# SebastianHafner/greedy_multimodal_learning

Measured on AMD Instinct MI355X. Metric: multi-view images/sec + step ms, ModelNet40 2-view MVCNN+MMTM @1/2/4/8 GPU, higher is better.
Workload: dtype bf16; 1 GPU; C2: 2-view MVCNN(ResNet-18 x2)+MMTM x3, guided gating (training_guided.gin eps 0.01, window 5, unlocked; decided on bf16-trunk gradients: d_BDR within ~6.5e-3 of eps may decide unlike fp32, INTEGRATION.md section 3); params=23773008, global_batch=64, per_gpu_batch=64, image=224, parallelism=dp1, hipgraph=True, device_gate=True

## Files before the change

greedy_multimodal_learning_amd/csrc/maxpool.hip:

```cpp
#include <type_traits>

#include "gm_common.h"

namespace gm {
namespace {

template <typename E>
__device__ __forceinline__ float round_to(float v) {
    if constexpr (std::is_same<E, uint16_t>::value) return __uint_as_float((uint32_t)Elem<uint16_t>::f2bf(v) << 16);
    else return v;
}

struct PoolArgs {
    int N, H, W, C8;
    int P, Q, k, s, pad;
    FastDiv fd_c8, fd_q, fd_p, fd_w, fd_h, fd_s;
    FastDiv fd_ng;
};

template <typename E, bool BNRELU = false>
__global__ __launch_bounds__(256) void k_maxpool_fwd(PoolArgs a, const void* __restrict__ x, void* __restrict__ y,
                                                     uint2* __restrict__ idx, const float* __restrict__ coef = nullptr,
                                                     void* __restrict__ xsel = nullptr) {
    const unsigned total = (unsigned)a.N * a.P * a.Q * a.C8;
    for (unsigned i = blockIdx.x * 256 + threadIdx.x; i < total; i += gridDim.x * 256) {
        unsigned t = a.fd_c8.div(i);
        const int cg = (int)(i - t * a.C8);
        unsigned t2 = a.fd_q.div(t);
        const int q = (int)(t - t2 * a.Q);
        const unsigned n_ = a.fd_p.div(t2);
        const int p = (int)(t2 - n_ * a.P);
        const int n = (int)n_;
        const int h0 = p * a.s - a.pad, w0 = q * a.s - a.pad;
        float m[8], xs[8];
        uint32_t ix[8];
        float sc[8], sh[8];
        if (BNRELU) {
            const float* cf = coef + (size_t)a.fd_ng.div((unsigned)n) * (a.C8 * 16);
            const float4* c4 = reinterpret_cast<const float4*>(cf + cg * 8);
            const float4* s4 = reinterpret_cast<const float4*>(cf + a.C8 * 8 + cg * 8);
            const float4 c0 = c4[0], c1 = c4[1], s0 = s4[0], s1 = s4[1];
            sc[0] = c0.x; sc[1] = c0.y; sc[2] = c0.z; sc[3] = c0.w; sc[4] = c1.x; sc[5] = c1.y; sc[6] = c1.z; sc[7] = c1.w;
            sh[0] = s0.x; sh[1] = s0.y; sh[2] = s0.z; sh[3] = s0.w; sh[4] = s1.x; sh[5] = s1.y; sh[6] = s1.z; sh[7] = s1.w;
        }
        const int hs = h0 < 0 ? 0 : h0, ws = w0 < 0 ? 0 : w0;
        const uint32_t first = (uint32_t)((hs - h0) * a.k + (ws - w0));
#pragma unroll
        for (int j = 0; j < 8; ++j) {
            m[j] = -__builtin_huge_valf();
            xs[j] = 0.f;
            ix[j] = first;
        }
        if (a.k == 3) {
            float v[9][8];
            const int xc = ((n * a.H + hs) * a.W + ws) * a.C8 + cg;
            const int x00 = xc + ((h0 - hs) * a.W + (w0 - ws)) * a.C8;
            const int WC8 = a.W * a.C8;
#pragma unroll
            for (int u = 0; u < 9; ++u) {
                const int h = h0 + u / 3, w = w0 + u % 3;
                const bool in = h >= 0 && h < a.H && w >= 0 && w < a.W;
                V8<E>::ld(x, in ? x00 + (u / 3) * WC8 + (u % 3) * a.C8 : xc, v[u]);
            }
#pragma unroll
            for (int u = 0; u < 9; ++u) {
                const int h = h0 + u / 3, w = w0 + u % 3;
                if (h < 0 || h >= a.H || w < 0 || w >= a.W) continue;
#pragma unroll
                for (int j = 0; j < 8; ++j) {
                    const float z = BNRELU ? round_to<E>(relu_nan(fmaf(v[u][j], sc[j], sh[j]))) : v[u][j];
                    if (z > m[j] || __builtin_isnan(z)) {
                        m[j] = z;
                        xs[j] = v[u][j];
                        ix[j] = (uint32_t)u;
                    }
                }
            }
        } else
        for (int r = 0; r < a.k; ++r) {
            const int h = h0 + r;
            if (h < 0 || h >= a.H) continue;
            for (int c = 0; c < a.k; ++c) {
                const int w = w0 + c;
                if (w < 0 || w >= a.W) continue;
                float v[8], raw[8];
                V8<E>::ld(x, (((long long)n * a.H + h) * a.W + w) * a.C8 + cg, v);
#pragma unroll
                for (int j = 0; j < 8; ++j) raw[j] = v[j];
                if (BNRELU) {
#pragma unroll
                    for (int j = 0; j < 8; ++j) v[j] = round_to<E>(relu_nan(fmaf(v[j], sc[j], sh[j])));
                }
                const uint32_t pos = (uint32_t)(r * a.k + c);
#pragma unroll
                for (int j = 0; j < 8; ++j) {
                    if (v[j] > m[j] || __builtin_isnan(v[j])) {
                        m[j] = v[j];
                        xs[j] = raw[j];
                        ix[j] = pos;
                    }
                }
            }
        }
        V8<E>::st(y, i, m);
        if (xsel) V8<E>::st(xsel, i, xs);
        idx[i] = make_uint2(ix[0] | ix[1] << 8 | ix[2] << 16 | ix[3] << 24, ix[4] | ix[5] << 8 | ix[6] << 16 | ix[7] << 24);
    }
}

template <typename E>
__global__ __launch_bounds__(256) void k_maxpool_bwd(PoolArgs a, const void* __restrict__ dy,
                                                     const uint2* __restrict__ idx, void* __restrict__ dx) {
    const unsigned total = (unsigned)a.N * a.H * a.W * a.C8;
    for (unsigned i = blockIdx.x * 256 + threadIdx.x; i < total; i += gridDim.x * 256) {
        unsigned t = a.fd_c8.div(i);
        const int cg = (int)(i - t * a.C8);
        unsigned t2 = a.fd_w.div(t);
        const int w = (int)(t - t2 * a.W);
        const unsigned n_ = a.fd_h.div(t2);
        const int h = (int)(t2 - n_ * a.H);
        const int n = (int)n_;
        int plo = h + a.pad - a.k + 1;
        plo = plo <= 0 ? 0 : (int)a.fd_s.div((unsigned)(plo + a.s - 1));
        int phi = (int)a.fd_s.div((unsigned)(h + a.pad));
        if (phi > a.P - 1) phi = a.P - 1;
        int qlo = w + a.pad - a.k + 1;
        qlo = qlo <= 0 ? 0 : (int)a.fd_s.div((unsigned)(qlo + a.s - 1));
        int qhi = (int)a.fd_s.div((unsigned)(w + a.pad));
        if (qhi > a.Q - 1) qhi = a.Q - 1;
        float g[8];
#pragma unroll
        for (int j = 0; j < 8; ++j) g[j] = 0.f;
        if (a.k == 3 && a.s == 2) {
            uint2 iv[4];
            float dv[4][8];
            bool ok[4];
            uint32_t pos[4];
#pragma unroll
            for (int u = 0; u < 4; ++u) {
                const int p = phi - 1 + (u >> 1), q = qhi - 1 + (u & 1);
                ok[u] = p >= plo && q >= qlo;
                const int pc = ok[u] ? p : phi, qc = ok[u] ? q : qhi;
                const long long o = (((long long)n * a.P + pc) * a.Q + qc) * a.C8 + cg;
                iv[u] = idx[o];
                V8<E>::ld(dy, o, dv[u]);
                pos[u] = (uint32_t)((h - (p * a.s - a.pad)) * a.k + (w - (q * a.s - a.pad)));
            }
#pragma unroll
            for (int u = 0; u < 4; ++u)
#pragma unroll
                for (int j = 0; j < 8; ++j) {
                    const uint32_t b = ((j < 4 ? iv[u].x : iv[u].y) >> (8 * (j & 3))) & 0xffu;
                    if (ok[u] && b == pos[u]) g[j] += dv[u][j];
                }
            V8<E>::st(dx, i, g);
            continue;
        }
        for (int p = plo; p <= phi; ++p) {
            for (int q = qlo; q <= qhi; ++q) {
                const long long o = (((long long)n * a.P + p) * a.Q + q) * a.C8 + cg;
                const uint2 iv = idx[o];
                const uint32_t pos = (uint32_t)((h - (p * a.s - a.pad)) * a.k + (w - (q * a.s - a.pad)));
                float d[8];
                V8<E>::ld(dy, o, d);
#pragma unroll
                for (int j = 0; j < 8; ++j) {
                    const uint32_t b = ((j < 4 ? iv.x : iv.y) >> (8 * (j & 3))) & 0xffu;
                    if (b == pos) g[j] += d[j];
                }
            }
        }
        V8<E>::st(dx, i, g);
    }
}

int prep(const gm_pool_desc* d, PoolArgs& a, const char* fn) {
    if (!d) {
        set_error("%s: null descriptor", fn);
        return GM_E_ARG;
    }
    if (d->N <= 0 || d->H <= 0 || d->W <= 0 || d->C <= 0 || d->C % 8 || d->k < 1 || d->k > 15 || d->stride < 1 ||
        d->pad < 0 || 2 * d->pad > d->k) {
        set_error("%s: unsupported N=%d H=%d W=%d C=%d k=%d s=%d pad=%d (C%%8==0, k<=15, pad<=k/2)", fn, d->N, d->H,
                  d->W, d->C, d->k, d->stride, d->pad);
        return GM_E_ARG;
    }
    a.N = d->N; a.H = d->H; a.W = d->W; a.C8 = d->C / 8;
    a.k = d->k; a.s = d->stride; a.pad = d->pad;
    a.P = (d->H + 2 * d->pad - d->k) / d->stride + 1;
    a.Q = (d->W + 2 * d->pad - d->k) / d->stride + 1;
    if (a.P <= 0 || a.Q <= 0) {
        set_error("%s: empty output", fn);
        return GM_E_ARG;
    }
    if ((long long)a.N * a.H * a.W * a.C8 >= (1ll << 31)) {
        set_error("%s: tensor too large (N*H*W*C/8 >= 2^31)", fn);
        return GM_E_ARG;
    }
    a.fd_c8 = FastDiv((uint32_t)a.C8);
    a.fd_q = FastDiv((uint32_t)a.Q);
    a.fd_p = FastDiv((uint32_t)a.P);
    a.fd_w = FastDiv((uint32_t)a.W);
    a.fd_h = FastDiv((uint32_t)a.H);
    a.fd_s = FastDiv((uint32_t)a.s);
    a.fd_ng = FastDiv((uint32_t)a.N);
    return GM_OK;
}

inline int grid_for(long long n) {
    long long g = (n + 255) / 256;
    if (g > 16384) g = 16384;
    return (int)(g < 1 ? 1 : g);
}

}
}

using namespace gm;

template <typename E>
int pool_fwd(const gm_pool_desc* d, const void* x, void* y, void* idx, void* stream, const char* fn) {
    PoolArgs a;
    int rc = prep(d, a, fn);
    if (rc) return rc;
    GM_REQUIRE(x && y && idx, "%s: null pointer", fn);
    const long long n = (long long)a.N * a.P * a.Q * a.C8;
    hipLaunchKernelGGL(k_maxpool_fwd<E>, dim3(grid_for(n)), dim3(256), 0, as_stream(stream), a, x, y,
                       static_cast<uint2*>(idx));
    return check_launch("k_maxpool_fwd");
}

template <typename E>
int pool_bwd(const gm_pool_desc* d, const void* dy, const void* idx, void* dx, void* stream, const char* fn) {
    PoolArgs a;
    int rc = prep(d, a, fn);
    if (rc) return rc;
    GM_REQUIRE(dy && idx && dx, "%s: null pointer", fn);
    const long long n = (long long)a.N * a.H * a.W * a.C8;
    hipLaunchKernelGGL(k_maxpool_bwd<E>, dim3(grid_for(n)), dim3(256), 0, as_stream(stream), a, dy,
                       static_cast<const uint2*>(idx), dx);
    return check_launch("k_maxpool_bwd");
}

extern "C" int gm_maxpool2d_fwd_bf16(const gm_pool_desc* d, const void* x, void* y, void* idx, void* stream) {
    return pool_fwd<uint16_t>(d, x, y, idx, stream, "gm_maxpool2d_fwd_bf16");
}

extern "C" int gm_bn_relu_maxpool2d_fwd_grouped_bf16(const gm_pool_desc* d, int G, const void* x, const float* coef,
                                                     void* y, void* idx, void* xsel, void* stream) {
    const char* fn = "gm_bn_relu_maxpool2d_fwd_grouped_bf16";
    GM_REQUIRE(d && G >= 1 && G <= 64, "%s: 1..64 groups", fn);
    gm_pool_desc dg = *d;
    dg.N = d->N * G;
    PoolArgs a;
    int rc = prep(&dg, a, fn);
    if (rc) return rc;
    a.fd_ng = FastDiv((uint32_t)d->N);
    GM_REQUIRE(x && coef && y && idx, "%s: null pointer", fn);
    const long long n = (long long)a.N * a.P * a.Q * a.C8;
    hipLaunchKernelGGL((k_maxpool_fwd<uint16_t, true>), dim3(grid_for(n)), dim3(256), 0, as_stream(stream), a, x, y,
                       static_cast<uint2*>(idx), coef, xsel);
    return check_launch("k_maxpool_fwd<bnrelu>");
}

extern "C" int gm_bn_relu_maxpool2d_fwd_bf16(const gm_pool_desc* d, const void* x, const float* coef, void* y,
                                             void* idx, void* stream) {
    return gm_bn_relu_maxpool2d_fwd_grouped_bf16(d, 1, x, coef, y, idx, nullptr, stream);
}

extern "C" int gm_maxpool2d_bwd_bf16(const gm_pool_desc* d, const void* dy, const void* idx, void* dx, void* stream) {
    return pool_bwd<uint16_t>(d, dy, idx, dx, stream, "gm_maxpool2d_bwd_bf16");
}

extern "C" int gm_maxpool2d_fwd_f32(const gm_pool_desc* d, const void* x, void* y, void* idx, void* stream) {
    return pool_fwd<float>(d, x, y, idx, stream, "gm_maxpool2d_fwd_f32");
}

extern "C" int gm_maxpool2d_bwd_f32(const gm_pool_desc* d, const void* dy, const void* idx, void* dx, void* stream) {
    return pool_bwd<float>(d, dy, idx, dx, stream, "gm_maxpool2d_bwd_f32");
}
```

Before: 36860 view-images/s.

## Add banded row-reuse kernel for fused BN-ReLU 3x3/s2 stem maxpool

Adds a specialized kernel for the fused BN+ReLU+maxpool forward (k=3, s=2, pad=1). Each thread handles a band of four output rows and carries the bottom input row of one output over as the top row of the next, which cuts redundant loads and normalization work. Comparisons are done on packed bf16 values with integer max and bit-select instructions, and a scalar exact path handles NaN and inf. The cost is fewer threads, since parallelism drops by the band factor, plus reliance on the bit patterns of non-negative bf16 values after ReLU for the ordering and tie-break to match the generic kernel.

```diff
diff --git a/greedy_multimodal_learning_amd/csrc/maxpool.hip b/greedy_multimodal_learning_amd/csrc/maxpool.hip
--- a/greedy_multimodal_learning_amd/csrc/maxpool.hip
+++ b/greedy_multimodal_learning_amd/csrc/maxpool.hip
@@ -108,6 +108,183 @@
     }
 }
 
+constexpr int kPoolBand = 4;
+
+struct RowArgs {
+    PoolArgs p;
+    int nb;
+    unsigned total;
+    FastDiv fd_nb;
+};
+
+typedef unsigned short us2 __attribute__((ext_vector_type(2)));
+typedef float f2 __attribute__((ext_vector_type(2)));
+typedef __bf16 bf2 __attribute__((ext_vector_type(2)));
+constexpr uint32_t kOne2 = 0x00010001u;
+
+__device__ __forceinline__ uint32_t pk_max(uint32_t a, uint32_t b) {
+    return __builtin_bit_cast(uint32_t,
+                              __builtin_elementwise_max(__builtin_bit_cast(us2, a), __builtin_bit_cast(us2, b)));
+}
+__device__ __forceinline__ uint32_t pk_sub(uint32_t a, uint32_t b) {
+    const us2 d = __builtin_bit_cast(us2, a) - __builtin_bit_cast(us2, b);
+    return __builtin_bit_cast(uint32_t, d);
+}
+__device__ __forceinline__ uint32_t pk_eq(uint32_t m1, uint32_t z) {
+    uint32_t r;
+    asm("v_pk_ashrrev_i16 %0, %1, %2" : "=v"(r) : "s"(15u * kOne2), "v"(pk_sub(m1, z)));
+    return r;
+}
+__device__ __forceinline__ uint32_t pk_sel(uint32_t mask, uint32_t a, uint32_t b) {
+    uint32_t r;
+    asm("v_bfi_b32 %0, %1, %2, %3" : "=v"(r) : "v"(mask), "v"(a), "v"(b));
+    return r;
+}
+
+struct RowRes {
+    uint32_t m[4], x[4], c[4];
+};
+
+__device__ __forceinline__ void rows_norm(const uint4 u, const f2* sc, const f2* sh, uint32_t* z) {
+    const uint32_t w[4] = {u.x, u.y, u.z, u.w};
+#pragma unroll
+    for (int k = 0; k < 4; ++k) {
+        f2 v = {bf_lo(w[k]), bf_hi(w[k])};
+        v = __builtin_elementwise_fma(v, sc[k], sh[k]);
+        v.x = relu_nan(v.x);
+        v.y = relu_nan(v.y);
+        z[k] = __builtin_bit_cast(uint32_t, __builtin_convertvector(v, bf2));
+    }
+}
+
+__device__ __forceinline__ void rows_scan(const uint4* v, uint32_t cl2, uint32_t cr2, const f2* sc, const f2* sh,
+                                          RowRes& r) {
+    uint32_t z0[4], z1[4], z2[4];
+    rows_norm(v[0], sc, sh, z0);
+    rows_norm(v[1], sc, sh, z1);
+    rows_norm(v[2], sc, sh, z2);
+    const uint32_t x0[4] = {v[0].x, v[0].y, v[0].z, v[0].w};
+    const uint32_t x1[4] = {v[1].x, v[1].y, v[1].z, v[1].w};
+    const uint32_t x2[4] = {v[2].x, v[2].y, v[2].z, v[2].w};
+#pragma unroll
+    for (int k = 0; k < 4; ++k) {
+        const uint32_t m = pk_max(pk_max(z0[k], z1[k]), z2[k]);
+        const uint32_t m1 = pk_sub(m, kOne2);
+        const uint32_t e0 = pk_eq(m1, z0[k]), e1 = pk_eq(m1, z1[k]);
+        r.m[k] = m;
+        r.x[k] = pk_sel(e0, x0[k], pk_sel(e1, x1[k], x2[k]));
+        r.c[k] = pk_sel(e0, cl2, pk_sel(e1, kOne2, cr2));
+    }
+}
+
+__device__ __forceinline__ void rows_window_exact(const PoolArgs& a, const uint4* __restrict__ x, int n, int p, int q,
+                                               int cg, const f2* sc, const f2* sh, uint32_t* mz, uint32_t* mx,
+                                               uint32_t* mpos) {
+    const int h0 = 2 * p - 1, w0 = 2 * q - 1;
+    const uint32_t first = (h0 < 0 ? 3u : 0u) + (w0 < 0 ? 1u : 0u);
+    float m[8], xr[8];
+    uint32_t ix[8];
+#pragma unroll
+    for (int j = 0; j < 8; ++j) {
+        m[j] = -__builtin_huge_valf();
+        xr[j] = 0.f;
+        ix[j] = first;
+    }
+#pragma unroll 1
+    for (int u = 0; u < 9; ++u) {
+        const int r = u / 3, c = u - 3 * r;
+        const int h = h0 + r, w = w0 + c;
+        if (h < 0 || h >= a.H || w < 0 || w >= a.W) continue;
+        float v[8];
+        V8<uint16_t>::ld(x, ((n * a.H + h) * a.W + w) * a.C8 + cg, v);
+#pragma unroll
+        for (int j = 0; j < 8; ++j) {
+            const float z = round_to<uint16_t>(relu_nan(fmaf(v[j], sc[j >> 1][j & 1], sh[j >> 1][j & 1])));
+            if (z > m[j] || __builtin_isnan(z)) {
+                m[j] = z;
+                xr[j] = v[j];
+                ix[j] = (uint32_t)u;
+            }
+        }
+    }
+#pragma unroll
+    for (int k = 0; k < 4; ++k) {
+        mz[k] = pack_bf2(m[2 * k], m[2 * k + 1]);
+        mx[k] = pack_bf2(xr[2 * k], xr[2 * k + 1]);
+        mpos[k] = ix[2 * k] | ix[2 * k + 1] << 16;
+    }
+}
+
+__global__ __launch_bounds__(256) void k_stem_pool_rows(RowArgs ra, const uint4* __restrict__ x,
+                                                        uint4* __restrict__ y, uint2* __restrict__ idx,
+                                                        const float* __restrict__ coef, uint4* __restrict__ xsel) {
+    const PoolArgs& a = ra.p;
+    const unsigned i = blockIdx.x * 256 + threadIdx.x;
+    if (i >= ra.total) return;
+    unsigned t = a.fd_c8.div(i);
+    const int cg = (int)(i - t * a.C8);
+    unsigned t2 = a.fd_q.div(t);
+    const int q = (int)(t - t2 * a.Q);
+    const unsigned n_ = ra.fd_nb.div(t2);
+    const int p0 = (int)(t2 - n_ * ra.nb) * kPoolBand;
+    const int p1 = p0 + kPoolBand < a.P ? p0 + kPoolBand : a.P;
+    const int n = (int)n_;
+    f2 sc[4], sh[4];
+    {
+        const float* cf = coef + (size_t)a.fd_ng.div((unsigned)n) * (a.C8 * 16);
+        const float4* c4 = reinterpret_cast<const float4*>(cf + cg * 8);
+        const float4* s4 = reinterpret_cast<const float4*>(cf + a.C8 * 8 + cg * 8);
+        const float4 c0 = c4[0], c1 = c4[1], s0 = s4[0], s1 = s4[1];
+        sc[0] = f2{c0.x, c0.y}; sc[1] = f2{c0.z, c0.w}; sc[2] = f2{c1.x, c1.y}; sc[3] = f2{c1.z, c1.w};
+        sh[0] = f2{s0.x, s0.y}; sh[1] = f2{s0.z, s0.w}; sh[2] = f2{s1.x, s1.y}; sh[3] = f2{s1.z, s1.w};
+    }
+    const bool vl = q > 0, vr = 2 * q + 1 < a.W;
+    const uint32_t cl2 = vl ? 0u : kOne2, cr2 = vr ? 2u * kOne2 : kOne2;
+    const int WC8 = a.W * a.C8;
+    const int oc = n * a.H * WC8 + 2 * q * a.C8 + cg;
+    const int ol = vl ? oc - a.C8 : oc, orr = vr ? oc + a.C8 : oc;
+
+    RowRes top;
+    bool tv = p0 > 0;
+    {
+        const int rb = (tv ? 2 * p0 - 1 : 0) * WC8;
+        const uint4 v[3] = {x[ol + rb], x[oc + rb], x[orr + rb]};
+        rows_scan(v, cl2, cr2, sc, sh, top);
+    }
+    int o = ((n * a.P + p0) * a.Q + q) * a.C8 + cg;
+    for (int p = p0; p < p1; ++p, o += a.Q * a.C8) {
+        const bool vb = 2 * p + 1 < a.H;
+        const int r1 = 2 * p * WC8, r2 = vb ? r1 + WC8 : r1;
+        const uint4 v1[3] = {x[ol + r1], x[oc + r1], x[orr + r1]};
+        const uint4 v2[3] = {x[ol + r2], x[oc + r2], x[orr + r2]};
+        RowRes mid, bot;
+        rows_scan(v1, cl2, cr2, sc, sh, mid);
+        rows_scan(v2, cl2, cr2, sc, sh, bot);
+        const uint32_t rt2 = tv ? 0u : 3u * kOne2, rb2 = vb ? 6u * kOne2 : 3u * kOne2;
+        uint32_t mz[4], mx[4], mpos[4];
+#pragma unroll
+        for (int k = 0; k < 4; ++k) {
+            const uint32_t m = pk_max(pk_max(top.m[k], mid.m[k]), bot.m[k]);
+            const uint32_t m1 = pk_sub(m, kOne2);
+            const uint32_t et = pk_eq(m1, top.m[k]), em = pk_eq(m1, mid.m[k]);
+            mz[k] = m;
+            mx[k] = pk_sel(et, top.x[k], pk_sel(em, mid.x[k], bot.x[k]));
+            mpos[k] = pk_sel(et, top.c[k] + rt2, pk_sel(em, mid.c[k] + 3u * kOne2, bot.c[k] + rb2));
+        }
+        top = bot;
+        tv = vb;
+        const uint32_t any = pk_max(pk_max(mz[0], mz[1]), pk_max(mz[2], mz[3]));
+        if ((any & 0xffffu) > 0x7f80u || (any >> 16) > 0x7f80u)
+            rows_window_exact(a, x, n, p, q, cg, sc, sh, mz, mx, mpos);
+        y[o] = make_uint4(mz[0], mz[1], mz[2], mz[3]);
+        if (xsel) xsel[o] = make_uint4(mx[0], mx[1], mx[2], mx[3]);
+        const uint32_t b0 = mpos[0] | mpos[0] >> 8, b1 = mpos[1] | mpos[1] >> 8;
+        const uint32_t b2 = mpos[2] | mpos[2] >> 8, b3 = mpos[3] | mpos[3] >> 8;
+        idx[o] = make_uint2((b0 & 0xffffu) | b1 << 16, (b2 & 0xffffu) | b3 << 16);
+    }
+}
+
+
 template <typename E>
 __global__ __launch_bounds__(256) void k_maxpool_bwd(PoolArgs a, const void* __restrict__ dy,
                                                      const uint2* __restrict__ idx, void* __restrict__ dx) {
@@ -257,6 +434,17 @@
     if (rc) return rc;
     a.fd_ng = FastDiv((uint32_t)d->N);
     GM_REQUIRE(x && coef && y && idx, "%s: null pointer", fn);
+    if (a.k == 3 && a.s == 2 && a.pad == 1) {
+        RowArgs ra;
+        ra.p = a;
+        ra.nb = (a.P + kPoolBand - 1) / kPoolBand;
+        ra.total = (unsigned)a.N * ra.nb * a.Q * a.C8;
+        ra.fd_nb = FastDiv((uint32_t)ra.nb);
+        hipLaunchKernelGGL(k_stem_pool_rows, dim3((ra.total + 255) / 256), dim3(256), 0, as_stream(stream), ra,
+                           static_cast<const uint4*>(x), static_cast<uint4*>(y), static_cast<uint2*>(idx), coef,
+                           static_cast<uint4*>(xsel));
+        return check_launch("k_stem_pool_rows");
+    }
     const long long n = (long long)a.N * a.P * a.Q * a.C8;
     hipLaunchKernelGGL((k_maxpool_fwd<uint16_t, true>), dim3(grid_for(n)), dim3(256), 0, as_stream(stream), a, x, y,
                        static_cast<uint2*>(idx), coef, xsel);
```

Result: no change. 37050 view-images/s, median of 6 (+0.5%).
